# Acelogic/Retrieval-based-Voice-Conversion-MLX

Hardware: AMD Instinct MI355X
Metric: audio-sec/sec (realtime factor) RVCv2 48kHz pipeline (higher is better)
Workload: dtype fp32-accurate (two-plane fp16 MFMA split); 1 GPU; C2: full RVCv2 48kHz pipeline, one 13.5 s utterance per step per GPU; samples_16k=216100, x_pad=1, f0_method=rmvpe, parallelism=dp1

## Files before the change

retrieval-based-voice-conversion-mlx_amd/csrc/capi.cpp:

```cpp
#include <algorithm>
#include <cmath>
#include <cstdio>
#include <cstdlib>
#include <cstring>
#include <string>
#include <unistd.h>
#include <vector>

#include "../../include/rvcx_test.h"
#include "runtime.h"

extern char** environ;

using namespace rvcx;

namespace rvcx {
static bool experimental_on() {
  const char* e = std::getenv("RVCX_EXPERIMENTAL");
  return e && std::atoi(e) == 1;
}
const char* rvcx_knob(const char* name) { return experimental_on() ? std::getenv(name) : nullptr; }
}

struct rvcx_ctx : public Ctx {};
// ... 967 lines not shown
      a.ldr = N;
      a.res_mode = RES_ADD_POST;
    }
    a.acc_mode = acc_mode == 0 ? ACC_STORE : (acc_mode == 1 ? ACC_ADD : ACC_ADD_DIV);
    a.acc_div = acc_div;
    a.math = 3;
    a.wsplit_fmt = WSPLIT_H16;
    a.w_static = 1;
    a.no_splitk = 1;
    if (!conv_wsb_eligible(a)) throw Error(RVCX_E_SHAPE, "rvcx_conv1d_gen: shape not eligible for the weight-streamed kernel");
    a.force_cfg = kernel == 1 ? conv_wsb_pick(a) : (kernel == 2 ? 40 : -1);
    a.wsplit_npad = conv_wsplit_npad(a.N);
    void* img = ctx->buf<char>("conv.test.wsplit", (size_t)conv_wsplit_bytes(a), static_cast<hipStream_t>(stream));
    check(conv_wsplit_build(a, img, static_cast<hipStream_t>(stream)), "conv_wsplit_build");
    a.wsplit = img;
    ConvArgs b = a;
    b.wsb = 1;
    if (kernel == 2 && !conv_wst_fits(b, false))
      throw Error(RVCX_E_SHAPE, "rvcx_conv1d_gen: shape not eligible for the weight-stationary kernel");
    launch_conv(*ctx, a, false, static_cast<hipStream_t>(stream), -1.0);
  });
}

int rvcx_conv1d_ex(rvcx_ctx* ctx, const rvcx_conv_test_desc* d, int* kind_out, int* ksplit_out, void* stream) {
  return guard(ctx, [&] {
    set_device(ctx);
    ctx->check_device_status();
    hipStream_t s = static_cast<hipStream_t>(stream);
    if (!d || !d->x || !d->w || !d->y || d->T_in <= 0 || d->C_in <= 0 || d->N <= 0 || d->taps <= 0 || d->dil <= 0 ||
        d->stride <= 0 || d->pad < 0 || d->T_out <= 0 || d->batch <= 0 || d->batch_inner <= 0 || d->ldx < d->C_in ||
        d->ldy < (d->gate_h > 0 ? d->gate_h : d->N) || d->pre_act < 0 || d->pre_act > ACT_LOGCLAMP || d->act < 0 ||
        d->act > ACT_LOGCLAMP || d->res_mode < RES_NONE || d->res_mode > RES_RSUB_POST || d->acc_mode < ACC_STORE ||
        d->acc_mode > ACC_ADD_DIV || (d->res_mode != RES_NONE && !d->res) || (d->res && d->ldr != 0 && d->ldr < d->N) ||
        d->route < 0 || d->route > 5 || d->gate_h < 0 || (d->gate_h > 0 && !d->gate_g) ||
        (d->ln_g && (!d->ln_b || !d->res)) ||
        (d->nz_har && (!d->nz_w || !d->nz_b || d->nz_C <= 0 || d->nz_u <= 0 || d->nz_stride <= 0)) ||
        ctx->is_weight(d->w))
      throw Error(RVCX_E_INVALID, "rvcx_conv1d_ex: bad argument");
    if ((int64_t)(d->T_out - 1) * d->stride + (int64_t)(d->taps - 1) * d->dil + 1 > d->T_in + 2 * (int64_t)d->pad)
      throw Error(RVCX_E_SHAPE, "rvcx_conv1d_ex: T_out exceeds the padded input");
    if ((int64_t)d->taps * d->N * d->C_in > INT32_MAX) throw Error(RVCX_E_SHAPE, "rvcx_conv1d_ex: size out of range");
    ConvArgs a;
    a.x = d->x; a.x_bs = d->x_bs; a.x_bs2 = d->x_bs2; a.ldx = d->ldx; a.T_in = d->T_in; a.C_in = d->C_in;
    a.pre_act = d->pre_act; a.pre_slope = d->pre_slope; a.pre_mask = d->pre_mask; a.pre_mask_bs = d->pre_mask_bs;
    a.w = d->w; a.ldw = d->C_in; a.w_ts = (long long)d->N * d->C_in; a.w_bs2 = d->w_bs2;
    a.taps = d->taps; a.stride = d->stride; a.dil = d->dil; a.pad = d->pad;
    a.y = d->y; a.y_bs = d->y_bs; a.y_bs2 = d->y_bs2; a.ldy = d->ldy; a.T_out = d->T_out; a.N = d->N;
    a.bias = d->bias; a.bias_bs2 = d->bias_bs2; a.alpha = d->alpha; a.act = d->act; a.slope = d->slope;
    a.res = d->res; a.res_bs = d->res_bs; a.res_bs2 = d->res_bs2; a.ldr = d->ldr; a.res_mode = d->res_mode;
    a.mask = d->mask; a.mask_bs = d->mask_bs; a.acc_mode = d->acc_mode; a.acc_div = d->acc_div;
    a.gate_h = d->gate_h; a.gate_g = d->gate_g; a.gate_g_bs = d->gate_g_bs;
    a.ln_g = d->ln_g; a.ln_b = d->ln_b; a.ln_eps = d->ln_eps;
    a.batch = d->batch; a.batch_inner = d->batch_inner;
    a.nz_har = d->nz_har; a.nz_bs = d->nz_bs; a.nz_stride = d->nz_stride; a.nz_kk = d->nz_kk; a.nz_u = d->nz_u;
    a.nz_C = d->nz_C; a.nz_w = d->nz_w; a.nz_b = d->nz_b;
    a.no_splitk = d->no_splitk ? 1 : 0;
    if (a.ln_g && (a.N > 1024 || a.batch_inner != 1 || a.res_mode != RES_NONE || a.acc_mode != ACC_STORE || a.gate_h > 0))
      throw Error(RVCX_E_SHAPE, "rvcx_conv1d_ex: the combine's LayerNorm takes N <= 1024, one group, no other residual");
    if (a.gate_h > 0 && (a.N != 2 * a.gate_h || a.batch_inner != 1 || a.act != ACT_NONE || a.alpha != 1.f || a.res ||
                         a.mask || a.acc_mode != ACC_STORE))
      throw Error(RVCX_E_SHAPE, "rvcx_conv1d_ex: the combine's gate takes N = 2 gate_h and no other epilogue field");
    if (a.nz_har && (a.nz_kk != 1 || a.N != a.nz_u * a.nz_C || a.gate_h > 0 || a.ln_g))
      throw Error(RVCX_E_SHAPE, "rvcx_conv1d_ex: the fused noise conv takes one tap and N = nz_u nz_C");
    int wsb = 0, expect = -1;
    if (d->route == 1 || d->route == 2) {
      a.math = d->route;
      expect = d->route == 1 ? CK_GEMM : CK_EMU;
    } else {
      a.w_static = 1;
      if (ctx->conv_math > 0) a.math = ctx->conv_math;
      if (d->route == 0) {
        wsb = conv_wsb_route(a, false);
      } else {
        a.math = 3;
        if (d->route == 3) {
          if (!conv_wsb_eligible(a)) throw Error(RVCX_E_SHAPE, "rvcx_conv1d_ex: form not eligible for the weight-streamed kernel");
          a.force_cfg = conv_wsb_pick(a);
          wsb = 1;
          expect = CK_WSB16;
        } else if (d->route == 4) {
          if (!conv_gs_eligible(a, false) || a.nz_har)
            throw Error(RVCX_E_SHAPE, "rvcx_conv1d_ex: form not eligible for the gather-streamed kernel");
          a.force_cfg = 30;
          wsb = 2;
          expect = CK_GS;
        } else {
          a.force_cfg = 40;
          wsb = 1;
          expect = CK_WST;
        }
      }
      if (wsb) {
        a.wsplit_fmt = conv_math_of(a) == 3 ? WSPLIT_H16 : WSPLIT_BF16;
        a.wsplit_npad = conv_wsplit_npad(a.N);
        void* img = ctx->buf<char>("conv.test.wsplit", (size_t)conv_wsplit_bytes(a), s);
        check(conv_wsplit_build(a, img, s), "conv_wsplit_build");
        a.wsplit = img;
      }
    }
    ConvArgs p = a;
    p.wsb = wsb;
    conv_plan_splitk(p, false);
    if (d->route == 5 && !conv_wst_fits(p, false))
      throw Error(RVCX_E_SHAPE, "rvcx_conv1d_ex: form not eligible for the weight-stationary kernel");
    if (!wsb && expect >= 0 && conv_unstreamed_kind(p) != expect)
      throw Error(RVCX_E_SHAPE, "rvcx_conv1d_ex: the dispatcher gives this shape to another kernel family");
    if ((a.gate_h > 0 || a.ln_g) && p.ksplit < 2)
      throw Error(RVCX_E_SHAPE, "rvcx_conv1d_ex: the gate / LayerNorm need a contraction that splits (two steps, no_splitk off)");
    if (a.nz_har && (wsb != 1 || p.ksplit > 1))
      throw Error(RVCX_E_SHAPE, "rvcx_conv1d_ex: the fused noise conv needs an unsplit weight-streamed / weight-stationary launch");
    if (ksplit_out) *ksplit_out = p.ksplit;
    launch_conv(*ctx, a, false, s, -1.0);
    if (kind_out) *kind_out = conv_last_kind();
  });
}

int rvcx_conv2d3x3(rvcx_ctx* ctx, const float* d_x, int H, int W, int C_in, const float* d_w, const float* d_bias,
                   int N, int act, int math, float* d_y, void* stream) {
// ... 449 lines not shown
```

retrieval-based-voice-conversion-mlx_amd/csrc/conv_dispatch.hip:

```cpp
#include <algorithm>
#include <cstdlib>
#include <string>

#include "conv_common.h"

namespace rvcx {

constexpr int CK = 32;

namespace {

inline int env_cfg(const char* name, int dflt) {
  const char* e = rvcx_knob(name);
  return e ? std::atoi(e) : dflt;
}
inline int conv_math(const ConvArgs& a) {
  static const int env = [] {
    const char* e = rvcx_knob("RVCX_CONV_MATH");
    if (e && (std::string(e) == "f32" || std::string(e) == "1")) return 1;
    if (e && (std::string(e) == "split" || std::string(e) == "2")) return 2;
    return 3;
  }();
  return a.math > 0 ? a.math : env;
}

template <bool TWO_D>
int pick_emu(const ConvArgs& a) {
  if (TWO_D) return a.N <= 32 ? 12 : 13;
  if (a.N <= 32) return a.taps >= 5 ? 12 : 1;
  if (a.taps >= 5) return 12;
  return 13;
}

template <bool TWO_D>
int pick_cfg(const ConvArgs& a) {
  if (a.force_cfg >= 0) return a.force_cfg;
  if (conv_math(a) >= 2) return pick_emu<TWO_D>(a);
  if (a.N <= 32) return 1;
  if (!TWO_D && a.taps >= 5) return 1;
  return 3;
}

inline void cfg_tile(int cfg, int& BM, int& BN) {
  if (conv_emu_tile(cfg, BM, BN)) return;
  static const int t[10][2] = {{256, 32}, {128, 32}, {128, 64}, {64, 64}, {128, 128}, {64, 128}, {256, 64},
                               {64, 64}, {128, 32}, {128, 128}};
  BM = t[cfg][0];
  BN = t[cfg][1];
}

inline int plan_rows(const ConvArgs& a) { return (a.plan_T > 0 && a.W_out <= 0) ? a.plan_T : a.T_out; }

inline int pick_wsb(const ConvArgs& a) {
  static const int c_long = env_cfg("RVCX_WCFG_LONG", 0);
  if (a.wsb == 2) return 30;
  if (a.N <= 32) return 24;
  if (a.taps <= 3 && a.N >= 1024 && plan_rows(a) >= 8192 && a.C_in < 512 && c_long == 0) return 25;
  if (a.taps <= 3) return 27;
  if (c_long > 0) return c_long;
  return (a.C_in < 256 && a.N >= 128) ? 25 : 23;
}
}
int conv_wsb_pick(const ConvArgs& a) {
  ConvArgs b = a;
  b.wsb = 1;
  return pick_wsb(b);
}
thread_local int g_conv_kind = CK_OTHER;
int conv_last_kind() { return g_conv_kind; }
const char* conv_kind_name(int k) {
  static const char* const names[CK_COUNT] = {"conv_wsb16_kernel", "conv_wsb_kernel", "conv_gs16_kernel",
                                              "conv_gsw16_kernel", "k_rb_pair", "k_conv2d_h16/k_conv2d_small",
                                              "conv_emu_kernel", "conv_gemm_kernel", "conv_tiny_kernel",
                                              "conv_wst16_kernel", "other"};
  return (k >= 0 && k < CK_COUNT) ? names[k] : "other";
}

namespace {

template <bool TWO_D>
hipError_t dispatch(const ConvArgs& a_in, hipStream_t s) {
  const ConvArgs& a = a_in;
  if (a.N <= 0 || a.T_out <= 0 || a.batch <= 0) return hipSuccess;
  if (a.C_in <= 0 || a.taps <= 0) return hipErrorInvalidValue;
  const bool nz = a.nz_har != nullptr;
  if (nz && (TWO_D || (a.ws && a.ksplit > 1) || a.nz_C <= 0 || a.nz_stride <= 0 ||
             a.nz_kk != 1 ||
             a.N != a.nz_u * a.nz_C || a.out_map != OUT_ROWS))
    return hipErrorInvalidValue;
  if ((a.gate_h > 0 || a.ln_g) && !(a.ws && a.ksplit > 1)) return hipErrorInvalidValue;
  if (tiny_fits(a)) {
    if (nz) return hipErrorInvalidValue;
    g_conv_kind = CK_TINY;
    return launch_tiny(a, TWO_D, s);
  }
  if (!nz && !(a.ws && a.ksplit > 1) && rows1x1_fits(a, TWO_D)) {
    g_conv_kind = CK_TINY;
    return launch_rows1x1(a, TWO_D, s);
  }
  if (a.wsb == 2 && a.wsplit && conv_math(a) >= 2 && conv_gs_eligible(a, TWO_D)) {
    const int ks = (a.ws && a.ksplit > 1) ? a.ksplit : 1;
    const int cfg = a.force_cfg >= 30 ? a.force_cfg : pick_wsb(a);
    g_conv_kind = (TWO_D && cfg == 30 && conv_gsw_eligible(a)) ? CK_GSW : CK_GS;
    hipError_t e = conv_gs_launch(a, cfg, s, TWO_D, ks);
    if (e == hipSuccess && ks > 1) e = launch_splitk_reduce(a, ks, TWO_D, s);
    if (e != hipErrorInvalidValue) return e;
  }
  if (a.wsb == 1 && a.wsplit && conv_math(a) >= 2 && conv_wsb_eligible(a, TWO_D)) {
    const int ks = (a.ws && a.ksplit > 1) ? a.ksplit : 1;
    if (ks == 1 && (a.force_cfg < 20 || a.force_cfg == 40) && conv_wst_fits(a, TWO_D)) {
      g_conv_kind = CK_WST;
      hipError_t e = conv_wst_launch(a, s);
      if (e != hipErrorInvalidValue) return e;
    }
    const int cfg = a.force_cfg >= 20 && a.force_cfg < 40 ? a.force_cfg : pick_wsb(a);
    g_conv_kind = CK_WSB16;
    hipError_t e = conv_wsb_launch(a, cfg, s, TWO_D, ks);
    if (e == hipSuccess && ks > 1) e = launch_splitk_reduce(a, ks, TWO_D, s);
    if (e != hipErrorInvalidValue) return e;
  }
  if (nz) return hipErrorInvalidValue;
  if (TWO_D && a.force_cfg < 0 && conv2d_small_fits(a)) {
    g_conv_kind = CK_SMALL2D;
    return conv2d_small(a, s);
  }
  const int cfg = pick_cfg<TWO_D>(a);
  const bool emu = cfg >= 10;
  g_conv_kind = emu ? CK_EMU : CK_GEMM;
  const bool gemm = !TWO_D && a.taps == 1 && a.stride == 1;
  const bool pipe = gemm && a.pipe >= 0;
  const int ksplit = (a.ws && a.ksplit > 1) ? a.ksplit : 1;
  auto run = [&](int c, bool p) -> hipError_t {
    hipError_t e = emu ? conv_emu_launch(a, c, TWO_D, p, ksplit, s) : conv_gemm_launch(a, c, TWO_D, p, ksplit, s);
    if (e != hipSuccess || ksplit == 1) return e;
    return launch_splitk_reduce(a, ksplit, TWO_D, s);
  };
  hipError_t e = run(cfg, pipe);
  if (e == hipErrorInvalidValue && pipe) e = run(cfg, false);
  if (e == hipErrorInvalidValue && a.force_cfg < 0) {
    for (int alt : {emu ? 13 : 3, emu ? 12 : 1}) {
      if (alt == cfg) continue;
      e = run(alt, false);
      if (e != hipErrorInvalidValue) break;
    }
  }
  return e;
}

}

long long conv_plan_splitk(ConvArgs& a, bool two_d) {
  a.ksplit = 1;
  if (a.N <= 0 || a.T_out <= 0 || a.no_splitk) return 0;
  if (tiny_fits(a)) return 0;
  if (two_d && a.force_cfg < 0 && conv2d_small_fits(a)) return 0;
  int BM, BN;
  if (a.wsb == 2) {
    conv_gs_tile(a.force_cfg >= 30 ? a.force_cfg : pick_wsb(a), BM, BN);
  } else if (a.wsb) {
    if (!conv_wsb_tile(a.force_cfg >= 20 ? a.force_cfg : pick_wsb(a), BM, BN)) return 0;
  } else {
    cfg_tile(two_d ? pick_cfg<true>(a) : pick_cfg<false>(a), BM, BN);
  }
  const int T_plan = two_d ? a.T_out : plan_rows(a);
  long long mtiles, mtiles_real;
  if (!two_d) {
    mtiles = (T_plan + BM - 1) / BM;
    mtiles_real = (a.T_out + BM - 1) / BM;
  } else {
    const int rw = a.W_out < BM ? a.W_out : BM;
    const int rh = BM / rw;
    mtiles = mtiles_real = (long long)((a.T_out + rh - 1) / rh) * ((a.W_out + rw - 1) / rw);
  }
  const long long tiles = mtiles * ((a.N + BN - 1) / BN) * a.batch * a.batch_inner;
  const long long tiles_real = mtiles_real * ((a.N + BN - 1) / BN) * a.batch * a.batch_inner;
  const int iters = ((a.C_in + CK - 1) / CK) * a.taps;
  const double M = two_d ? (double)a.T_out * a.W_out : (double)T_plan;
  const double flops = 2.0 * M * a.N * (double)a.C_in * a.taps * a.batch * a.batch_inner;
  static const int target = env_cfg("RVCX_SPLITK_TARGET", 512);
  constexpr int min_tiles = 192;
  constexpr int min_iters = 4;
  const bool combine_epi = a.gate_h > 0 || a.ln_g;
  if (!combine_epi && (tiles >= min_tiles || iters < min_iters || (flops < 1.0e8 && iters < 16))) return 0;
  int ks = (int)((target + tiles - 1) / tiles);
  constexpr int gs_min_steps = 8;
  ks = std::min(ks, a.wsb == 2 ? iters / gs_min_steps : iters / 2);
  ks = std::min(ks, 32);
  if (a.wsb == 2 && two_d && (a.force_cfg < 0 || a.force_cfg == 30) && conv_gsw_eligible(a))
    ks = std::min(ks, (a.C_in + CK - 1) / CK);
  if (combine_epi && iters >= 2) ks = std::max(ks, 2);
  if (ks < 2) return 0;
// ... 31 lines not shown
```

retrieval-based-voice-conversion-mlx_amd/csrc/conv_gs.hip:

```cpp
#include <algorithm>
#include <cstdlib>

#include "conv_common.h"
#include "split_bf16.h"

namespace rvcx {

namespace {

using namespace splitbf16;

constexpr int GS_BLK = 1024;
#ifndef GS_DEPTH
#define GS_DEPTH 3
#endif
constexpr int GS_D = GS_DEPTH;

template <int TN16>
__device__ __forceinline__ void mma_h16(const bf16x8 (&af)[2], const bf16x8 (&bf)[TN16][2], f32x4 (&acc)[TN16],
                                        f32x4 (&acc2)[TN16]) {
  const f16x8 ah = __builtin_bit_cast(f16x8, af[0]), al = __builtin_bit_cast(f16x8, af[1]);
#pragma unroll
  for (int tn = 0; tn < TN16; ++tn) {
    const f16x8 bh = __builtin_bit_cast(f16x8, bf[tn][0]);
    acc[tn] = __builtin_amdgcn_mfma_f32_16x16x32_f16(ah, bh, acc[tn], 0, 0, 0);
    f32x4 c = acc2[tn];
    c = __builtin_amdgcn_mfma_f32_16x16x32_f16(al, bh, c, 0, 0, 0);
    c = __builtin_amdgcn_mfma_f32_16x16x32_f16(ah, __builtin_bit_cast(f16x8, bf[tn][1]), c, 0, 0, 0);
    acc2[tn] = c;
  }
}
template <int TM16, int TN16, int WN>
__device__ __forceinline__ void h16_finish(const char* wsp, size_t tail_off, int n0, f32x4 (&acc)[TM16][TN16],
                                           const f32x4 (&acc2)[TM16][TN16]) {
  const int wn = (threadIdx.x >> 6) % WN;
  const float* inv = reinterpret_cast<const float*>(wsp + tail_off) + n0 + wn * TN16 * 16 + (threadIdx.x & 15);
#pragma unroll
  for (int tn = 0; tn < TN16; ++tn) {
    const float iv = inv[tn * 16];
#pragma unroll
    for (int tm = 0; tm < TM16; ++tm)
#pragma unroll
      for (int r = 0; r < 4; ++r) acc[tm][tn][r] = (acc[tm][tn][r] + acc2[tm][tn][r] * H16_LO_INV) * iv;
  }
}

template <int BM, int BN, int WM, int WN, bool TWO_D, int MODE>
__global__ __launch_bounds__(CONV_THREADS, 2) void conv_gs16_kernel(const ConvArgs a, const char* __restrict__ wsp,
                                                                    const int Npad, const int ntn, const int ksplit,
                                                                    const int mfast) {
  constexpr int NT = CONV_THREADS;
  constexpr int TM16 = BM / (WM * 16);
  constexpr int TN16 = BN / (WN * 16);
  constexpr int AV = BM * EC4 / NT;
  constexpr int PA = MODE & 3;
  constexpr bool PMASK = !TWO_D && (MODE & 4) != 0;
  constexpr bool H16 = (MODE & 16) != 0;
  constexpr int NQ = H16 ? 2 : 3;
  constexpr int RS = H16 ? ERS_H : ERS;
  static_assert(WM * WN == 4 && TM16 >= 1 && TN16 >= 1 && BM * EC4 % NT == 0, "tile shape");
  extern __shared__ __attribute__((aligned(16))) char smem_gs[];

  const int tid = threadIdx.x;
  const int lane = tid & 63;
  const int wave = tid >> 6;
  const int wm = wave / WN, wn = wave % WN;
  const int lc = lane & 15, lg = lane >> 4;
  int bx, by, bz;
  conv_block_coords(ntn, bx, by, bz);
  if (mfast && ntn > 0) {
    const int t = bx * ntn + by;
    const int mt = (int)gridDim.x / ntn;
    bx = t % mt;
    by = t / mt;
  }
  const int zsplit = bz % ksplit;
  const int b = bz / ksplit;
  const int n0 = by * BN;
// ... 398 lines not shown
  const int ntn = ntiles;
  dim3 grid((unsigned)(mtiles * ntiles), 1, a.batch * ksplit);
  const bool h16 = a.wsplit_fmt == WSPLIT_H16;
  const size_t smem = (size_t)(rh + 2) * (W + 2) * (h16 ? ERS_H : ERS);
  const double wbytes = 6.0 * a.N * a.C_in * 9, abytes = 4.0 * (double)a.T_out * W * a.C_in * a.batch;
  const int mfast = wbytes > abytes ? 1 : 0;
  switch (pre_mode(a.pre_act) | (h16 ? 16 : 0)) {
    case 0: launch_gsw_mode<0>(a, grid, smem, ntn, ksplit, mfast, s); break;
    case 1: launch_gsw_mode<1>(a, grid, smem, ntn, ksplit, mfast, s); break;
    case 2: launch_gsw_mode<2>(a, grid, smem, ntn, ksplit, mfast, s); break;
    case 16: launch_gsw_mode<16>(a, grid, smem, ntn, ksplit, mfast, s); break;
    case 17: launch_gsw_mode<17>(a, grid, smem, ntn, ksplit, mfast, s); break;
    default: launch_gsw_mode<18>(a, grid, smem, ntn, ksplit, mfast, s); break;
  }
  return hipGetLastError();
}

}

bool conv_gs_eligible(const ConvArgs& a, bool two_d) {
  const bool vec_a = ((a.ldx & 3) == 0) && ((reinterpret_cast<uintptr_t>(a.x) & 15) == 0) && ((a.x_bs & 3) == 0);
  const bool up2d = two_d && a.out_map == OUT_UPSAMPLE2D && a.out_cv > 0 && a.N == 4 * a.out_cv && !a.res &&
                    a.acc_mode == ACC_STORE && !a.mask && !a.nz_har;
  const bool common = a.batch_inner == 1 && !a.b_kn && a.C_in % EK == 0 && a.C_in > 0 && a.taps >= 1 && vec_a &&
                      (a.out_map == OUT_ROWS || up2d) && a.stride >= 1 && a.dil >= 1;
  if (!common) return false;
  const long long rows_in = two_d ? (long long)a.T_in * a.W_in : a.T_in;
  if (rows_in * a.ldx + a.C_in >= INT32_MAX) return false;
  if (!two_d) return (long long)a.T_out * a.stride < INT32_MAX / 2 && a.T_in < INT32_MAX / 2;
  return a.taps == a.KH * a.KW && !a.pre_mask && a.stride == 1 && a.W_out >= 1 && a.W_in >= 1;
}

bool conv_gs_tile(int cfg, int& BM, int& BN) {
  if (cfg != 30) return false;
  BM = 64;
  BN = 64;
  return true;
}

bool conv_gsw_eligible(const ConvArgs& a) {
  return conv_gs_eligible(a, true) && a.KH == 3 && a.KW == 3 && a.padh == 1 && a.padw == 1 &&
         a.T_in == a.T_out && a.W_in == a.W_out && a.W_out <= GSW_MAXW && GSW_MAXW % a.W_out == 0 && a.W_out >= 4;
}

hipError_t conv_gs_launch(const ConvArgs& a, int cfg, hipStream_t s, bool two_d, int ksplit) {
  if (!a.wsplit || !conv_gs_eligible(a, two_d) || a.lowp) return hipErrorInvalidValue;
  if (cfg != 30) return hipErrorInvalidValue;
  if (two_d && conv_gsw_eligible(a)) return launch_gsw(a, ksplit, s);
  return two_d ? launch_gs<64, 64, 2, 2, true>(a, ksplit, s)
               : launch_gs<64, 64, 2, 2, false>(a, ksplit, s);
}

}
```

retrieval-based-voice-conversion-mlx_amd/csrc/rvcx_kernels.h:

```cpp
#pragma once
#include <hip/hip_runtime.h>
#include <cstdint>

namespace rvcx {

const char* rvcx_knob(const char* name);

enum Act : int {
  ACT_NONE = 0,
  ACT_LRELU = 1,
  ACT_RELU = 2,
  ACT_GELU = 3,
  ACT_TANH = 4,
  ACT_SIGMOID = 5,
  ACT_LOGCLAMP = 6,
};

enum ResMode : int {
  RES_NONE = 0,
  RES_ADD_PRE = 1,
  RES_ADD_POST = 2,
  RES_RSUB_POST = 3,
};

// ... 87 lines not shown
                      CK_OTHER, CK_COUNT };
int conv_last_kind();
const char* conv_kind_name(int k);
int conv_math_of(const ConvArgs& a);
int conv_unstreamed_kind(const ConvArgs& a);
hipError_t conv2d(const ConvArgs& a, hipStream_t s);
bool conv2d_small_fits(const ConvArgs& a);
hipError_t conv2d_small(const ConvArgs& a, hipStream_t s);
long long small2d_wsplit_bytes(const ConvArgs& a);
hipError_t small2d_wsplit_build(const ConvArgs& a, void* out, hipStream_t s);
long long conv_plan_splitk(ConvArgs& a, bool two_d);

hipError_t fill(float* p, float v, long long n, hipStream_t s);
hipError_t transpose_bct_btc(const float* x, float* y, int B, int C, int T, hipStream_t s);
hipError_t transpose_btc_bct(const float* x, float* y, int B, int T, int C, int ldx, hipStream_t s);
hipError_t channel_flip(const float* x, float* y, int rows, int C, hipStream_t s);
hipError_t gather_rows(const float* table, int ld_table, const int32_t* idx, float* y, int rows, int C,
                       hipStream_t s);
hipError_t seq_mask(const int32_t* lengths, float* mask, int B, int T, hipStream_t s);
hipError_t upconv_phase_pack(const float* w, int C, int co, float* out, hipStream_t s);
hipError_t layernorm_rows(const float* x, const float* r, float* y, const float* gamma, const float* beta,
                          int rows, int D, float eps, const float* mask, hipStream_t s);
hipError_t gate_tanh_sigmoid(const float* xin, int ldx, const float* g, long long g_bs, float* acts, int B,
                             int T, int H, hipStream_t s);
bool conv_wsb_eligible(const ConvArgs& a, bool two_d = false);
bool conv_wsb_wants(const ConvArgs& a);
int conv_wsb_route(const ConvArgs& a, bool two_d);
bool conv_wsb_tile(int cfg, int& BM, int& BN);
int conv_wsb_pick(const ConvArgs& a);
bool conv_gs_eligible(const ConvArgs& a, bool two_d);
bool conv_gsw_eligible(const ConvArgs& a);
bool conv_gs_tile(int cfg, int& BM, int& BN);
hipError_t conv_gs_launch(const ConvArgs& a, int cfg, hipStream_t s, bool two_d, int ksplit);
int conv_wsplit_npad(int N);
long long conv_wsplit_bytes(const ConvArgs& a);
hipError_t conv_wsplit_build(const ConvArgs& a, void* out, hipStream_t s);
hipError_t conv_wsb_launch(const ConvArgs& a, int cfg, hipStream_t s, bool two_d = false,
                           int ksplit = 1);
bool conv_wst_fits(const ConvArgs& a, bool two_d);
hipError_t conv_wst_launch(const ConvArgs& a, hipStream_t s);
struct RbPairArgs {
  const float* x = nullptr;
  long long x_bs = 0;
  const void* w1s = nullptr;
  const float* b1 = nullptr;
  const void* w2s = nullptr;
  const float* b2 = nullptr;
  int C = 0, k = 0, d = 1, T = 0, B = 1;
  float* y = nullptr;
  long long y_bs = 0;
  int acc_mode = ACC_STORE;
  float acc_div = 1.f;
  int wfmt = 0;
  int lowp = 0;
};
enum RbWfmt : int { RB_WBF16 = 0, RB_WF16 = 1 };
bool rb_pair_fits(int C, int k, int d);
long long rb_wsplit_bytes(int C, int k, int wfmt = RB_WBF16);
hipError_t rb_wsplit_build(const float* w, int C, int k, void* out, hipStream_t s, int wfmt = RB_WBF16);
hipError_t rb_pair(const RbPairArgs& a, int cfg, hipStream_t s);
int flash_attn_splits(int B, int nh, int T);
long long flash_attn_ws_floats(int B, int nh, int T, int dk, int nsplit);
hipError_t flash_attn(const float* qkv, int ldq, int B, int T, int nh, int dk, float qscale, const float* rel_k,
                      const float* rel_v, int window, const float* mask, float* part_o, float* part_ml, int nsplit,
                      float* out, int ldo, hipStream_t s);
hipError_t crepe_frames(const float* audio, long long n, long long f_first, int nf, float* out, int ld, hipStream_t s,
// ... 170 lines not shown
```

retrieval-based-voice-conversion-mlx_amd/csrc/split_bf16.h:

```cpp
#pragma once
#include "conv_common.h"

namespace rvcx {
namespace splitbf16 {

typedef __bf16 bf16x8 __attribute__((ext_vector_type(8)));
typedef __bf16 bf16x2 __attribute__((ext_vector_type(2)));
typedef float f32x2 __attribute__((ext_vector_type(2)));

constexpr int EK = 32;
constexpr int EC4 = EK / 4;
constexpr int PLANE = EK * 2;
constexpr int ERS = 3 * PLANE + 16;

__device__ __forceinline__ unsigned pk_bf16(float x, float y) {
  const bf16x2 h = __builtin_convertvector((f32x2){x, y}, bf16x2);
  return __builtin_bit_cast(unsigned, h);
}
__device__ __forceinline__ float lo_f(unsigned p) { return __uint_as_float(p << 16); }
__device__ __forceinline__ float hi_f(unsigned p) { return __uint_as_float(p & 0xffff0000u); }

__device__ __forceinline__ void put_split4(char* row, int c4, f32x4 v) {
  uint2 h, m, l;
  h.x = pk_bf16(v[0], v[1]);
// ... 32 lines not shown
  const f16x2 h = __builtin_convertvector((f32x2){x, y}, f16x2);
  return __builtin_bit_cast(unsigned, h);
}
__device__ __forceinline__ float f16lo_f(unsigned p) { return (float)__builtin_bit_cast(f16x2, p)[0]; }
__device__ __forceinline__ float f16hi_f(unsigned p) { return (float)__builtin_bit_cast(f16x2, p)[1]; }

__device__ __forceinline__ void absmax_wave_publish(float m, unsigned* dst) {
  for (int o = 32; o > 0; o >>= 1) m = fmaxf(m, __shfl_xor(m, o));
  if ((threadIdx.x & 63) == 0) atomicMax(dst, __float_as_uint(m));
}
__device__ __forceinline__ float h16_weight_scale(unsigned mbits) {
  const float m = __uint_as_float(mbits);
  int e = 0;
  (void)frexpf(m, &e);
  return m > 0.f ? ldexpf(1.f, 8 - e) : 1.f;
}

template <int NPL>
__device__ __forceinline__ void put_h16x4(char* row, int c4, f32x4 v) {
  uint2 h;
  h.x = pk_f16(v[0], v[1]);
  h.y = pk_f16(v[2], v[3]);
  *reinterpret_cast<uint2*>(row + c4 * 2) = h;
  if constexpr (NPL > 1) {
    uint2 l;
    l.x = pk_f16((v[0] - f16lo_f(h.x)) * H16_LO, (v[1] - f16hi_f(h.x)) * H16_LO);
    l.y = pk_f16((v[2] - f16lo_f(h.y)) * H16_LO, (v[3] - f16hi_f(h.y)) * H16_LO);
    *reinterpret_cast<uint2*>(row + PLANE + c4 * 2) = l;
  }
}

__device__ __forceinline__ int store_row(int w) { return (w & ~7) | (((w & 7) >> 1) + 4 * (w & 1)); }


}
}
```

retrieval-based-voice-conversion-mlx_amd/rvcx/engine.py:

```python
from __future__ import annotations

import ctypes
from typing import Dict, Mapping, Optional

import numpy as np

from . import _lib
from .config import SYNTH_48K_V2, SynthConfig
from .weights import normalize_state


def _ptr(t) -> Optional[int]:
    return None if t is None else t.data_ptr()


class Engine:

    def __init__(self, device: int = 0):
        import torch

        self.lib = _lib.load()
        if not torch.cuda.is_available():
            raise RuntimeError("rvcx needs a ROCm GPU: torch.cuda.is_available() is False")
        self.torch = torch
# ... 690 lines not shown
        b = self._dev(bias, torch.float32) if bias is not None else None
        T = int(x.shape[0])
        T_out = (T + 2 * padding - dilation * (K - 1) - 1) // stride + 1
        y = torch.empty((T_out, N), dtype=torch.float32, device=self.device)
        m = {"default": 0, "f32": 1, "split": 2, "wsb": 3, "gs": 4, "h16": 5, "f16": 6, "gs_h16": 7}[math]
        self._check(self.lib.rvcx_conv1d(self.ctx, _ptr(x), T, C, _ptr(wk), _ptr(b), N, K, dilation, padding, stride,
                                         m, _ptr(y), T_out, self.stream()), "conv1d")
        return y

    def conv1d_gen(self, x, w, bias=None, dilation: int = 1, padding: int = 0, pre_slope: float = 0.1,
                   slope=None, res=None, acc=None, acc_mode: int = 0, acc_div: float = 1.0,
                   kernel: str = "policy"):
        torch = self.torch
        x = self._dev(x, torch.float32)
        w = torch.as_tensor(w, dtype=torch.float32)
        N, C, K = (int(v) for v in w.shape)
        wk = self._dev(w.permute(2, 0, 1).contiguous(), torch.float32)
        b = self._dev(bias, torch.float32) if bias is not None else None
        r = self._dev(res, torch.float32) if res is not None else None
        T = int(x.shape[0])
        T_out = T + 2 * padding - dilation * (K - 1)
        if acc is not None:
            y = self._dev(acc, torch.float32).clone()
        else:
            y = torch.empty((T_out, N), dtype=torch.float32, device=self.device)
        kn = {"policy": 0, "wsb": 1, "wst": 2}[kernel]
        self._check(self.lib.rvcx_conv1d_gen(self.ctx, _ptr(x), T, C, _ptr(wk), _ptr(b), N, K, dilation, padding,
                                             0 if pre_slope is None else 1,
                                             0.0 if pre_slope is None else float(pre_slope), 0 if slope is None else 1,
                                             0.0 if slope is None else float(slope), _ptr(r), int(acc_mode),
                                             float(acc_div), kn, _ptr(y), self.stream()), "conv1d_gen")
        return y

    ROUTES = {"policy": 0, "f32": 1, "emu": 2, "wsb": 3, "gs": 4, "wst": 5}

    def conv1d_ex(self, x, w, y, *, T_in: int, C_in: int, N: int, T_out: int, ldx: int, ldy: int, taps: int = 1,
                  dil: int = 1, pad: int = 0, stride: int = 1, ldr: int = 0, bias=None, res=None, mask=None,
                  pre_mask=None, batch: int = 1, x_bs: int = 0, y_bs: int = 0, res_bs: int = 0, mask_bs: int = 0,
                  pre_mask_bs: int = 0, batch_inner: int = 1, x_bs2: int = 0, w_bs2: int = 0, y_bs2: int = 0,
                  res_bs2: int = 0, bias_bs2: int = 0, pre_act: int = 0, pre_slope: float = 0.0, act: int = 0,
                  slope: float = 0.0, alpha: float = 1.0, res_mode: int = 0, acc_mode: int = 0, acc_div: float = 1.0,
                  gate_h: int = 0, gate_g=None, gate_g_bs: int = 0, ln_g=None, ln_b=None, ln_eps: float = 1e-5,
                  nz_har=None, nz_bs: int = 0, nz_stride: int = 0, nz_kk: int = 0, nz_u: int = 1, nz_C: int = 0,
                  nz_w=None, nz_b=None, route="policy", no_splitk: bool = False):
        torch = self.torch
        G, B, i64 = int(batch_inner), int(batch), int

        def span(t, name, last):
            if t is None:
                return None
            if not (isinstance(t, torch.Tensor) and t.dtype == torch.float32 and t.device == self.device):
                raise ValueError(f"conv1d_ex: {name} must be a float32 tensor on {self.device}")
            room = t.untyped_storage().nbytes() // 4 - t.storage_offset()
            if last < 0 or last >= room:
                raise ValueError(f"conv1d_ex: {name} addresses element {last}, its storage holds {room} from the view")
            return t.data_ptr()

        ncol = gate_h if gate_h > 0 else N
        d = _lib.ConvTestDesc()
        d.x = span(x, "x", (B - 1) * x_bs + (G - 1) * x_bs2 + (T_in - 1) * ldx + C_in - 1)
        d.w = span(w, "w", (G - 1) * w_bs2 + taps * N * C_in - 1)
        d.y = span(y, "y", (B - 1) * y_bs + (G - 1) * y_bs2 + (T_out - 1) * ldy + ncol - 1)
        d.bias = span(bias, "bias", (G - 1) * bias_bs2 + N - 1)
        d.res = span(res, "res", (B - 1) * res_bs + (G - 1) * res_bs2 + (T_out - 1) * ldr + N - 1)
        d.mask = span(mask, "mask", (B - 1) * mask_bs + T_out - 1)
        d.pre_mask = span(pre_mask, "pre_mask", (B - 1) * pre_mask_bs + T_in - 1)
        d.gate_g = span(gate_g, "gate_g", (B - 1) * gate_g_bs + N - 1)
# ... 102 lines not shown
```

Measured before the change: 1154 audio-sec/sec.

## Add wave-split-K gather-streamed conv kernel for small-tile-count convolutions

Adds a new gather-streamed conv kernel that splits the reduction (channel×tap) dimension across the four waves of a block and combines the partial accumulators through shared memory before the epilogue. The dispatcher picks it by default for 1D fp32-split convs with N≤192 and at most 256 output tiles, and turns off block-level split-K for those shapes. The aim is better occupancy and latency on small, under-parallelised convs, where the old 64x64 tile left most of the GPU idle. The cost is an LDS reduction and extra shared memory per block, plus a new test route.

```diff
diff --git a/retrieval-based-voice-conversion-mlx_amd/csrc/capi.cpp b/retrieval-based-voice-conversion-mlx_amd/csrc/capi.cpp
--- a/retrieval-based-voice-conversion-mlx_amd/csrc/capi.cpp
+++ b/retrieval-based-voice-conversion-mlx_amd/csrc/capi.cpp
@@ -1023,7 +1023,7 @@
         d->ldy < (d->gate_h > 0 ? d->gate_h : d->N) || d->pre_act < 0 || d->pre_act > ACT_LOGCLAMP || d->act < 0 ||
         d->act > ACT_LOGCLAMP || d->res_mode < RES_NONE || d->res_mode > RES_RSUB_POST || d->acc_mode < ACC_STORE ||
         d->acc_mode > ACC_ADD_DIV || (d->res_mode != RES_NONE && !d->res) || (d->res && d->ldr != 0 && d->ldr < d->N) ||
-        d->route < 0 || d->route > 5 || d->gate_h < 0 || (d->gate_h > 0 && !d->gate_g) ||
+        d->route < 0 || d->route > 6 || d->gate_h < 0 || (d->gate_h > 0 && !d->gate_g) ||
         (d->ln_g && (!d->ln_b || !d->res)) ||
         (d->nz_har && (!d->nz_w || !d->nz_b || d->nz_C <= 0 || d->nz_u <= 0 || d->nz_stride <= 0)) ||
         ctx->is_weight(d->w))
@@ -1075,6 +1075,13 @@
           a.force_cfg = 30;
           wsb = 2;
           expect = CK_GS;
+        } else if (d->route == 6) {
+          a.wsplit_fmt = WSPLIT_H16;
+          if (!conv_gsk_eligible(a) || a.nz_har)
+            throw Error(RVCX_E_SHAPE, "rvcx_conv1d_ex: form not eligible for the wave-split-K gather-streamed kernel");
+          a.force_cfg = conv_gsk_cfg();
+          wsb = 2;
+          expect = CK_GS;
         } else {
           a.force_cfg = 40;
           wsb = 1;
diff --git a/retrieval-based-voice-conversion-mlx_amd/csrc/conv_dispatch.hip b/retrieval-based-voice-conversion-mlx_amd/csrc/conv_dispatch.hip
--- a/retrieval-based-voice-conversion-mlx_amd/csrc/conv_dispatch.hip
+++ b/retrieval-based-voice-conversion-mlx_amd/csrc/conv_dispatch.hip
@@ -51,9 +51,21 @@
 
 inline int plan_rows(const ConvArgs& a) { return (a.plan_T > 0 && a.W_out <= 0) ? a.plan_T : a.T_out; }
 
+inline int pick_gs(const ConvArgs& a) {
+  static const int force = env_cfg("RVCX_GSK", -1);
+  const bool can = a.W_out <= 0 && conv_math(a) == 3 && !a.lowp && (!a.wsplit || a.wsplit_fmt == WSPLIT_H16);
+  if (!can || force == 0) return 30;
+  if (force > 30) return conv_gsk_cfg();
+  if (a.gate_h > 0 || a.ln_g || a.N > 192) return 30;
+  if (a.C_in == a.N && (a.N == 64 || a.N == 128) && (a.taps == 2 || a.taps == 3)) return 30;
+  int BM, BN;
+  conv_gsk_tile(conv_gsk_cfg(), BM, BN);
+  const long long tiles = (long long)((plan_rows(a) + BM - 1) / BM) * ((a.N + BN - 1) / BN) * a.batch * a.batch_inner;
+  return tiles <= 256 ? conv_gsk_cfg() : 30;
+}
 inline int pick_wsb(const ConvArgs& a) {
   static const int c_long = env_cfg("RVCX_WCFG_LONG", 0);
-  if (a.wsb == 2) return 30;
+  if (a.wsb == 2) return pick_gs(a);
   if (a.N <= 32) return 24;
   if (a.taps <= 3 && a.N >= 1024 && plan_rows(a) >= 8192 && a.C_in < 512 && c_long == 0) return 25;
   if (a.taps <= 3) return 27;
@@ -100,7 +112,8 @@
   }
   if (a.wsb == 2 && a.wsplit && conv_math(a) >= 2 && conv_gs_eligible(a, TWO_D)) {
     const int ks = (a.ws && a.ksplit > 1) ? a.ksplit : 1;
-    const int cfg = a.force_cfg >= 30 ? a.force_cfg : pick_wsb(a);
+    int cfg = a.force_cfg >= 30 ? a.force_cfg : pick_wsb(a);
+    if (a.force_cfg < 30 && cfg > 30 && (TWO_D || !conv_gsk_eligible(a))) cfg = 30;
     g_conv_kind = (TWO_D && cfg == 30 && conv_gsw_eligible(a)) ? CK_GSW : CK_GS;
     hipError_t e = conv_gs_launch(a, cfg, s, TWO_D, ks);
     if (e == hipSuccess && ks > 1) e = launch_splitk_reduce(a, ks, TWO_D, s);
@@ -156,7 +169,9 @@
   if (two_d && a.force_cfg < 0 && conv2d_small_fits(a)) return 0;
   int BM, BN;
   if (a.wsb == 2) {
-    conv_gs_tile(a.force_cfg >= 30 ? a.force_cfg : pick_wsb(a), BM, BN);
+    const int cfg = a.force_cfg >= 30 ? a.force_cfg : pick_wsb(a);
+    conv_gs_tile(cfg, BM, BN);
+    if (a.force_cfg < 30 && cfg > 30 && !(a.gate_h > 0 || a.ln_g)) return 0;
   } else if (a.wsb) {
     if (!conv_wsb_tile(a.force_cfg >= 20 ? a.force_cfg : pick_wsb(a), BM, BN)) return 0;
   } else {
diff --git a/retrieval-based-voice-conversion-mlx_amd/csrc/conv_gs.hip b/retrieval-based-voice-conversion-mlx_amd/csrc/conv_gs.hip
--- a/retrieval-based-voice-conversion-mlx_amd/csrc/conv_gs.hip
+++ b/retrieval-based-voice-conversion-mlx_amd/csrc/conv_gs.hip
@@ -10,40 +10,10 @@
 
 using namespace splitbf16;
 
-constexpr int GS_BLK = 1024;
 #ifndef GS_DEPTH
 #define GS_DEPTH 3
 #endif
 constexpr int GS_D = GS_DEPTH;
-
-template <int TN16>
-__device__ __forceinline__ void mma_h16(const bf16x8 (&af)[2], const bf16x8 (&bf)[TN16][2], f32x4 (&acc)[TN16],
-                                        f32x4 (&acc2)[TN16]) {
-  const f16x8 ah = __builtin_bit_cast(f16x8, af[0]), al = __builtin_bit_cast(f16x8, af[1]);
-#pragma unroll
-  for (int tn = 0; tn < TN16; ++tn) {
-    const f16x8 bh = __builtin_bit_cast(f16x8, bf[tn][0]);
-    acc[tn] = __builtin_amdgcn_mfma_f32_16x16x32_f16(ah, bh, acc[tn], 0, 0, 0);
-    f32x4 c = acc2[tn];
-    c = __builtin_amdgcn_mfma_f32_16x16x32_f16(al, bh, c, 0, 0, 0);
-    c = __builtin_amdgcn_mfma_f32_16x16x32_f16(ah, __builtin_bit_cast(f16x8, bf[tn][1]), c, 0, 0, 0);
-    acc2[tn] = c;
-  }
-}
-template <int TM16, int TN16, int WN>
-__device__ __forceinline__ void h16_finish(const char* wsp, size_t tail_off, int n0, f32x4 (&acc)[TM16][TN16],
-                                           const f32x4 (&acc2)[TM16][TN16]) {
-  const int wn = (threadIdx.x >> 6) % WN;
-  const float* inv = reinterpret_cast<const float*>(wsp + tail_off) + n0 + wn * TN16 * 16 + (threadIdx.x & 15);
-#pragma unroll
-  for (int tn = 0; tn < TN16; ++tn) {
-    const float iv = inv[tn * 16];
-#pragma unroll
-    for (int tm = 0; tm < TM16; ++tm)
-#pragma unroll
-      for (int r = 0; r < 4; ++r) acc[tm][tn][r] = (acc[tm][tn][r] + acc2[tm][tn][r] * H16_LO_INV) * iv;
-  }
-}
 
 template <int BM, int BN, int WM, int WN, bool TWO_D, int MODE>
 __global__ __launch_bounds__(CONV_THREADS, 2) void conv_gs16_kernel(const ConvArgs a, const char* __restrict__ wsp,
@@ -508,6 +478,7 @@
 }
 
 bool conv_gs_tile(int cfg, int& BM, int& BN) {
+  if (conv_gsk_tile(cfg, BM, BN)) return true;
   if (cfg != 30) return false;
   BM = 64;
   BN = 64;
@@ -521,6 +492,7 @@
 
 hipError_t conv_gs_launch(const ConvArgs& a, int cfg, hipStream_t s, bool two_d, int ksplit) {
   if (!a.wsplit || !conv_gs_eligible(a, two_d) || a.lowp) return hipErrorInvalidValue;
+  if (cfg > 30) return two_d ? hipErrorInvalidValue : conv_gsk_launch(a, cfg, s, ksplit);
   if (cfg != 30) return hipErrorInvalidValue;
   if (two_d && conv_gsw_eligible(a)) return launch_gsw(a, ksplit, s);
   return two_d ? launch_gs<64, 64, 2, 2, true>(a, ksplit, s)
diff --git a/retrieval-based-voice-conversion-mlx_amd/csrc/conv_gsk.hip b/retrieval-based-voice-conversion-mlx_amd/csrc/conv_gsk.hip
--- /dev/null
+++ b/retrieval-based-voice-conversion-mlx_amd/csrc/conv_gsk.hip
@@ -0,0 +1,265 @@
+#include <algorithm>
+#include <cstdlib>
+
+#include "conv_common.h"
+#include "split_bf16.h"
+
+namespace rvcx {
+
+namespace {
+
+using namespace splitbf16;
+
+#ifndef GSK_DEPTH
+#define GSK_DEPTH 2
+#endif
+constexpr int GSK_D = GSK_DEPTH;
+
+__device__ __forceinline__ void split_h16x8(const f32x4& v0, const f32x4& v1, bf16x8 (&af)[2]) {
+  uint4 h, l;
+  h.x = pk_f16(v0[0], v0[1]);
+  h.y = pk_f16(v0[2], v0[3]);
+  h.z = pk_f16(v1[0], v1[1]);
+  h.w = pk_f16(v1[2], v1[3]);
+  l.x = pk_f16((v0[0] - f16lo_f(h.x)) * H16_LO, (v0[1] - f16hi_f(h.x)) * H16_LO);
+  l.y = pk_f16((v0[2] - f16lo_f(h.y)) * H16_LO, (v0[3] - f16hi_f(h.y)) * H16_LO);
+  l.z = pk_f16((v1[0] - f16lo_f(h.z)) * H16_LO, (v1[1] - f16hi_f(h.z)) * H16_LO);
+  l.w = pk_f16((v1[2] - f16lo_f(h.w)) * H16_LO, (v1[3] - f16hi_f(h.w)) * H16_LO);
+  af[0] = __builtin_bit_cast(bf16x8, h);
+  af[1] = __builtin_bit_cast(bf16x8, l);
+}
+
+template <int BM, int BN, int KG, int WN, int MODE>
+__global__ __launch_bounds__(CONV_THREADS, 2) void conv_gsk16_kernel(const ConvArgs a, const char* __restrict__ wsp,
+                                                                     const int Npad, const int ntn, const int ksplit,
+                                                                     const int mfast) {
+  constexpr int TM16 = BM / 16;
+  constexpr int TN16 = BN / (WN * 16);
+  constexpr int PA = MODE & 3;
+  constexpr bool PMASK = (MODE & 4) != 0;
+  constexpr int D = GSK_D;
+  constexpr int EWM = BM >= 64 ? 2 : 1, EWN = 4 / EWM;
+  constexpr int ETM = BM / (EWM * 16), ETN = BN / (EWN * 16);
+  static_assert(KG * WN == 4 && TM16 >= 1 && TN16 >= 1 && ETM >= 1 && ETN >= 1 && D >= 2, "tile shape");
+  extern __shared__ __attribute__((aligned(16))) char smem_gsk[];
+
+  const int tid = threadIdx.x;
+  const int lane = tid & 63;
+  const int wave = __builtin_amdgcn_readfirstlane(tid >> 6);
+  const int kg = wave / WN, wn = wave % WN;
+  const int lc = lane & 15, lg = lane >> 4;
+  int bx, by, bz;
+  conv_block_coords(ntn, bx, by, bz);
+  if (mfast && ntn > 0) {
+    const int t = bx * ntn + by;
+    const int mt = (int)gridDim.x / ntn;
+    bx = t % mt;
+    by = t / mt;
+  }
+  const int zsplit = bz % ksplit;
+  const int b = bz / ksplit;
+  const int n0 = by * BN;
+  const int m0 = bx * BM;
+  const float* X = a.x + (long long)b * a.x_bs + 8 * lg;
+  const float* PM = PMASK ? a.pre_mask + (long long)b * a.pre_mask_bs : nullptr;
+
+  const int taps = a.taps;
+  const int total = (a.C_in / EK) * taps;
+  const int per = (total + ksplit - 1) / ksplit;
+  const int it0 = zsplit * per, it1 = min(total, it0 + per);
+  const int pg = (max(it1 - it0, 0) + KG - 1) / KG;
+  const int s0 = it0 + kg * pg, s1 = min(it1, s0 + pg);
+  const int last = s1 - 1;
+
+  int g0[TM16];
+  unsigned rokb = 0u;
+#pragma unroll
+  for (int tm = 0; tm < TM16; ++tm) {
+    const int m = m0 + tm * 16 + lc;
+    rokb |= m < a.T_out ? (1u << tm) : 0u;
+    g0[tm] = m * a.stride - a.pad;
+  }
+  int a_st = s0, a_ch = s0 / taps, a_tap = s0 - (s0 / taps) * taps;
+  f32x4 ar[D][TM16][2];
+  float am[D][TM16];
+  unsigned aok[D];
+  auto load_a = [&](f32x4 (&dst)[TM16][2], float (&dm)[TM16], unsigned& okb) __attribute__((always_inline)) {
+    const float* src = X + a_ch * EK;
+    const int sh = a_tap * a.dil;
+    okb = 0u;
+#pragma unroll
+    for (int tm = 0; tm < TM16; ++tm) {
+      const int g = g0[tm] + sh;
+      const bool ok = ((rokb >> tm) & 1u) && (unsigned)g < (unsigned)a.T_in;
+      const unsigned gc = ok ? (unsigned)g : 0u;
+      const float* p = src + gc * (unsigned)a.ldx;
+      dst[tm][0] = *reinterpret_cast<const f32x4*>(p);
+      dst[tm][1] = *reinterpret_cast<const f32x4*>(p + 4);
+      if constexpr (PMASK) dm[tm] = PM[gc];
+      okb |= ok ? (1u << tm) : 0u;
+    }
+    if (a_st < last) {
+      ++a_st;
+      if (++a_tap == taps) {
+        a_tap = 0;
+        ++a_ch;
+      }
+    }
+  };
+
+  typedef bf16x8 BFrag[TN16][2];
+  BFrag br[D];
+  const char* bp = wsp + (size_t)((n0 + wn * TN16 * 16) >> 4) * (2 * GS_BLK) + lane * 16;
+  const size_t bstep = (size_t)Npad * 2 * PLANE;
+  auto load_b = [&](int st, BFrag& dst) __attribute__((always_inline)) {
+    const char* p = bp + (size_t)st * bstep;
+#pragma unroll
+    for (int tn = 0; tn < TN16; ++tn)
+#pragma unroll
+      for (int q = 0; q < 2; ++q) dst[tn][q] = *reinterpret_cast<const bf16x8*>(p + tn * (2 * GS_BLK) + q * GS_BLK);
+  };
+
+  f32x4 acc[TM16][TN16], acc2[TM16][TN16];
+#pragma unroll
+  for (int tm = 0; tm < TM16; ++tm)
+#pragma unroll
+    for (int tn = 0; tn < TN16; ++tn) {
+      acc[tm][tn] = f32x4{0.f, 0.f, 0.f, 0.f};
+      acc2[tm][tn] = f32x4{0.f, 0.f, 0.f, 0.f};
+    }
+  auto compute = [&](const f32x4 (&src)[TM16][2], const float (&sm)[TM16], unsigned okb, const BFrag& bf)
+      __attribute__((always_inline)) {
+#pragma unroll
+    for (int tm = 0; tm < TM16; ++tm) {
+      f32x4 v[2] = {src[tm][0], src[tm][1]};
+      const bool ok = (okb >> tm) & 1u;
+#pragma unroll
+      for (int h = 0; h < 2; ++h) {
+#pragma unroll
+        for (int j = 0; j < 4; ++j) v[h][j] = pre_fn<PA>(v[h][j], a.pre_act, a.pre_slope);
+        if constexpr (PMASK) {
+#pragma unroll
+          for (int j = 0; j < 4; ++j) v[h][j] = ok ? v[h][j] * sm[tm] : 0.f;
+        } else {
+#pragma unroll
+          for (int j = 0; j < 4; ++j) v[h][j] = ok ? v[h][j] : 0.f;
+        }
+#pragma unroll
+        for (int j = 0; j < 4; ++j) v[h][j] *= H16_XS;
+      }
+      bf16x8 af[2];
+      split_h16x8(v[0], v[1], af);
+      mma_h16(af, bf, acc[tm], acc2[tm]);
+    }
+  };
+
+  if (s0 < s1) {
+    auto clampst = [&](int st) { return st < last ? st : last; };
+#pragma unroll
+    for (int p = 0; p < D - 1; ++p) {
+      load_a(ar[p], am[p], aok[p]);
+      load_b(clampst(s0 + p), br[p]);
+    }
+    auto step = [&](int i, int p) __attribute__((always_inline)) {
+      load_a(ar[(p + D - 1) % D], am[(p + D - 1) % D], aok[(p + D - 1) % D]);
+      load_b(clampst(i + D - 1), br[(p + D - 1) % D]);
+      __builtin_amdgcn_sched_barrier(0);
+      compute(ar[p], am[p], aok[p], br[p]);
+    };
+    int base = s0;
+    for (; base + D <= s1; base += D) {
+#pragma unroll
+      for (int p = 0; p < D; ++p) step(base + p, p);
+    }
+#pragma unroll
+    for (int p = 0; p < D - 1; ++p)
+      if (base + p < s1) step(base + p, p);
+  }
+
+  f32x4* P = reinterpret_cast<f32x4*>(smem_gsk);
+#pragma unroll
+  for (int tm = 0; tm < TM16; ++tm)
+#pragma unroll
+    for (int tn = 0; tn < TN16; ++tn) {
+      P[(((wave * TM16 + tm) * TN16 + tn) * 2 + 0) * 64 + lane] = acc[tm][tn];
+      P[(((wave * TM16 + tm) * TN16 + tn) * 2 + 1) * 64 + lane] = acc2[tm][tn];
+    }
+  __syncthreads();
+  f32x4 e[ETM][ETN], e2[ETM][ETN];
+  const int ewm = wave / EWN, ewn = wave % EWN;
+#pragma unroll
+  for (int tm = 0; tm < ETM; ++tm)
+#pragma unroll
+    for (int tn = 0; tn < ETN; ++tn) {
+      const int rb = ewm * ETM + tm, cb = ewn * ETN + tn;
+      const int kwn = cb / TN16, ktn = cb % TN16;
+      f32x4 s = P[((((0 * WN + kwn) * TM16 + rb) * TN16 + ktn) * 2 + 0) * 64 + lane];
+      f32x4 s2 = P[((((0 * WN + kwn) * TM16 + rb) * TN16 + ktn) * 2 + 1) * 64 + lane];
+#pragma unroll
+      for (int g = 1; g < KG; ++g) {
+        s += P[((((g * WN + kwn) * TM16 + rb) * TN16 + ktn) * 2 + 0) * 64 + lane];
+        s2 += P[((((g * WN + kwn) * TM16 + rb) * TN16 + ktn) * 2 + 1) * 64 + lane];
+      }
+      e[tm][tn] = s;
+      e2[tm][tn] = s2;
+    }
+  h16_finish<ETM, ETN, EWN>(wsp, (size_t)total * bstep, n0, e, e2);
+  store_tile16<ETM, ETN, EWM, EWN>(a, m0, n0, b, zsplit, ksplit, a.T_out, e);
+}
+
+template <int BM, int BN, int KG, int WN, int MODE>
+void launch_gsk_mode(const ConvArgs& a, dim3 grid, size_t smem, int ntn, int ksplit, int mfast, hipStream_t s) {
+  static size_t smem_set = 64 * 1024;
+  if (smem > smem_set) {
+    (void)hipFuncSetAttribute(reinterpret_cast<const void*>(conv_gsk16_kernel<BM, BN, KG, WN, MODE>),
+                              hipFuncAttributeMaxDynamicSharedMemorySize, (int)smem);
+    smem_set = smem;
+  }
+  hipLaunchKernelGGL((conv_gsk16_kernel<BM, BN, KG, WN, MODE>), grid, dim3(CONV_THREADS), smem, s, a,
+                     static_cast<const char*>(a.wsplit), a.wsplit_npad, ntn, ksplit, mfast);
+}
+
+template <int BM, int BN, int KG, int WN>
+hipError_t launch_gsk(const ConvArgs& a, int ksplit, hipStream_t s) {
+  const long long mtiles = ((long long)a.T_out + BM - 1) / BM;
+  if (mtiles > INT32_MAX / 64 || a.wsplit_npad % BN != 0 || ksplit < 1 || (ksplit > 1 && !a.ws)) return hipErrorInvalidValue;
+  const int ntiles = (a.N + BN - 1) / BN;
+  const int ntn = ntiles;
+  dim3 grid((unsigned)(mtiles * ntiles), 1, a.batch * ksplit);
+  constexpr size_t base = (size_t)4 * (BM / 16) * (BN / (WN * 16)) * 2 * 64 * 16;
+  const size_t smem = std::min(base + (size_t)std::max(0, a.lds_pad), std::max(base, (size_t)160 * 1024));
+  const double wbytes = 4.0 * a.N * a.C_in * a.taps, abytes = 4.0 * (double)a.T_out * a.C_in * a.batch;
+  const int mfast = wbytes > abytes ? 1 : 0;
+  switch (pre_mode(a.pre_act) | (a.pre_mask ? 4 : 0)) {
+    case 0: launch_gsk_mode<BM, BN, KG, WN, 0>(a, grid, smem, ntn, ksplit, mfast, s); break;
+    case 1: launch_gsk_mode<BM, BN, KG, WN, 1>(a, grid, smem, ntn, ksplit, mfast, s); break;
+    case 2: launch_gsk_mode<BM, BN, KG, WN, 2>(a, grid, smem, ntn, ksplit, mfast, s); break;
+    case 4: launch_gsk_mode<BM, BN, KG, WN, 4>(a, grid, smem, ntn, ksplit, mfast, s); break;
+    case 5: launch_gsk_mode<BM, BN, KG, WN, 5>(a, grid, smem, ntn, ksplit, mfast, s); break;
+    case 6: launch_gsk_mode<BM, BN, KG, WN, 6>(a, grid, smem, ntn, ksplit, mfast, s); break;
+    default: return hipErrorInvalidValue;
+  }
+  return hipGetLastError();
+}
+
+}
+
+bool conv_gsk_eligible(const ConvArgs& a) {
+  return conv_gs_eligible(a, false) && a.W_out <= 0 && a.wsplit_fmt == WSPLIT_H16 && !a.lowp;
+}
+
+bool conv_gsk_tile(int cfg, int& BM, int& BN) {
+  if (cfg != 31) return false;
+  BM = 32;
+  BN = 64;
+  return true;
+}
+
+int conv_gsk_cfg() { return 31; }
+
+hipError_t conv_gsk_launch(const ConvArgs& a, int cfg, hipStream_t s, int ksplit) {
+  if (!a.wsplit || !conv_gsk_eligible(a) || cfg != 31) return hipErrorInvalidValue;
+  return launch_gsk<32, 64, 4, 1>(a, ksplit, s);
+}
+
+}
diff --git a/retrieval-based-voice-conversion-mlx_amd/csrc/rvcx_kernels.h b/retrieval-based-voice-conversion-mlx_amd/csrc/rvcx_kernels.h
--- a/retrieval-based-voice-conversion-mlx_amd/csrc/rvcx_kernels.h
+++ b/retrieval-based-voice-conversion-mlx_amd/csrc/rvcx_kernels.h
@@ -143,6 +143,10 @@
 bool conv_gsw_eligible(const ConvArgs& a);
 bool conv_gs_tile(int cfg, int& BM, int& BN);
 hipError_t conv_gs_launch(const ConvArgs& a, int cfg, hipStream_t s, bool two_d, int ksplit);
+bool conv_gsk_eligible(const ConvArgs& a);
+bool conv_gsk_tile(int cfg, int& BM, int& BN);
+int conv_gsk_cfg();
+hipError_t conv_gsk_launch(const ConvArgs& a, int cfg, hipStream_t s, int ksplit);
 int conv_wsplit_npad(int N);
 long long conv_wsplit_bytes(const ConvArgs& a);
 hipError_t conv_wsplit_build(const ConvArgs& a, void* out, hipStream_t s);
diff --git a/retrieval-based-voice-conversion-mlx_amd/csrc/split_bf16.h b/retrieval-based-voice-conversion-mlx_amd/csrc/split_bf16.h
--- a/retrieval-based-voice-conversion-mlx_amd/csrc/split_bf16.h
+++ b/retrieval-based-voice-conversion-mlx_amd/csrc/split_bf16.h
@@ -88,6 +88,36 @@
 
 __device__ __forceinline__ int store_row(int w) { return (w & ~7) | (((w & 7) >> 1) + 4 * (w & 1)); }
 
+constexpr int GS_BLK = 1024;
+
+template <int TN16>
+__device__ __forceinline__ void mma_h16(const bf16x8 (&af)[2], const bf16x8 (&bf)[TN16][2], f32x4 (&acc)[TN16],
+                                        f32x4 (&acc2)[TN16]) {
+  const f16x8 ah = __builtin_bit_cast(f16x8, af[0]), al = __builtin_bit_cast(f16x8, af[1]);
+#pragma unroll
+  for (int tn = 0; tn < TN16; ++tn) {
+    const f16x8 bh = __builtin_bit_cast(f16x8, bf[tn][0]);
+    acc[tn] = __builtin_amdgcn_mfma_f32_16x16x32_f16(ah, bh, acc[tn], 0, 0, 0);
+    f32x4 c = acc2[tn];
+    c = __builtin_amdgcn_mfma_f32_16x16x32_f16(al, bh, c, 0, 0, 0);
+    c = __builtin_amdgcn_mfma_f32_16x16x32_f16(ah, __builtin_bit_cast(f16x8, bf[tn][1]), c, 0, 0, 0);
+    acc2[tn] = c;
+  }
+}
+template <int TM16, int TN16, int WN>
+__device__ __forceinline__ void h16_finish(const char* wsp, size_t tail_off, int n0, f32x4 (&acc)[TM16][TN16],
+                                           const f32x4 (&acc2)[TM16][TN16]) {
+  const int wn = (threadIdx.x >> 6) % WN;
+  const float* inv = reinterpret_cast<const float*>(wsp + tail_off) + n0 + wn * TN16 * 16 + (threadIdx.x & 15);
+#pragma unroll
+  for (int tn = 0; tn < TN16; ++tn) {
+    const float iv = inv[tn * 16];
+#pragma unroll
+    for (int tm = 0; tm < TM16; ++tm)
+#pragma unroll
+      for (int r = 0; r < 4; ++r) acc[tm][tn][r] = (acc[tm][tn][r] + acc2[tm][tn][r] * H16_LO_INV) * iv;
+  }
+}
 
 }
 }
diff --git a/retrieval-based-voice-conversion-mlx_amd/rvcx/engine.py b/retrieval-based-voice-conversion-mlx_amd/rvcx/engine.py
--- a/retrieval-based-voice-conversion-mlx_amd/rvcx/engine.py
+++ b/retrieval-based-voice-conversion-mlx_amd/rvcx/engine.py
@@ -746,7 +746,7 @@
                                              float(acc_div), kn, _ptr(y), self.stream()), "conv1d_gen")
         return y
 
-    ROUTES = {"policy": 0, "f32": 1, "emu": 2, "wsb": 3, "gs": 4, "wst": 5}
+    ROUTES = {"policy": 0, "f32": 1, "emu": 2, "wsb": 3, "gs": 4, "wst": 5, "gsk": 6}
 
     def conv1d_ex(self, x, w, y, *, T_in: int, C_in: int, N: int, T_out: int, ldx: int, ldy: int, taps: int = 1,
                   dil: int = 1, pad: int = 0, stride: int = 1, ldr: int = 0, bias=None, res=None, mask=None,
```

After: 1156 audio-sec/sec, median of 4. No clear change (+0.1%).
